# Cogito2012/OpenTAL

Hardware: AMD Instinct MI355X
Metric: clips/sec training step, 256-frame THUMOS14 clips (higher is better)
Workload: dtype bf16

## Files before the change

opental_amd/csrc/conv_gemm.hip:

```cpp
#include "common.h"
#include "conv_index.h"
#include "conv_select.h"
#include <cstdlib>
#include <cstring>
#include <mutex>
#include <type_traits>

#ifndef OTAL_CONV_PART
#define OTAL_CONV_PART 0
#endif

#include "conv1a_tile.h"
namespace otal_conv {
struct ConvArgs;
__attribute__((visibility("hidden"))) int launch_half(int mode, int kernel, int cw, ConvArgs& a, void* ws, size_t ws_bytes, hipStream_t st);
}

namespace {

constexpr int NT = 256;
enum { EPI_RELU = 1, EPI_ACCUM = 2, NO_STORE = 8, NO_BARRIER = 16, EPI_NPAD8 = 32 };

typedef float f32x16 __attribute__((ext_vector_type(16)));

// ... 573 lines not shown
                    pk.y = pack_bf16x2(rb[8 * h + 2], rb[8 * h + 3]);
                    pk.z = pack_bf16x2(rb[8 * h + 4], rb[8 * h + 5]);
                    pk.w = pack_bf16x2(rb[8 * h + 6], rb[8 * h + 7]);
                    *reinterpret_cast<uint4*>(Bs + b_n * KP + b_kq * B_PER + 8 * h) = pk;
                }
            }
        }
    };

    constexpr int WAVES_N = BN / (32 * WN);
    const int wm0 = (wave / WAVES_N) * (32 * WM);
    const int wn0 = (wave % WAVES_N) * (32 * WN);
    f32x16 acc[WM][WN];
#pragma unroll
    for (int i = 0; i < WM; ++i)
#pragma unroll
        for (int j = 0; j < WN; ++j)
#pragma unroll
            for (int r = 0; r < 16; ++r) acc[i][j][r] = 0.f;

    const int nk = (k_end - k_begin + BK - 1) / BK;
    prep(k_begin, nk > 0);
#pragma unroll
    for (int q = 0; q < A_LOADS; ++q) loadA(q, k_begin, nk > 0);
#pragma unroll
    for (int q = 0; q < B_LOADS; ++q) loadB(q, k_begin, nk > 0);
    store_tiles(0);
    __syncthreads();
    constexpr int NCH = PREC ? 2 : 8;
    constexpr int A_PER_CH = (A_LOADS + NCH - 1) / NCH, B_PER_CH = (B_LOADS + NCH - 1) / NCH;
    for (int it = 0; it < nk; ++it) {
        const int buf = it & 1;
        const bool has_next = it + 1 < nk;
        const int kn = k_begin + (it + 1) * BK;
        prep(kn, has_next);
#pragma unroll
        for (int c = 0; c < NCH; ++c) {
#pragma unroll
            for (int q = 0; q < A_PER_CH; ++q)
                if (c * A_PER_CH + q < A_LOADS) loadA(c * A_PER_CH + q, kn, has_next);
#pragma unroll
            for (int q = 0; q < B_PER_CH; ++q)
                if (c * B_PER_CH + q < B_LOADS) loadB(c * B_PER_CH + q, kn, has_next);
            if constexpr (PREC == 0) {
                const float* as = reinterpret_cast<const float*>(smemA[buf]);
                const float* bs = reinterpret_cast<const float*>(smemB[buf]);
                float av[WM], bv[WN];
                const int kr = 2 * c + (lane >> 5);
#pragma unroll
                for (int i = 0; i < WM; ++i) av[i] = as[kr * LDA + wm0 + i * 32 + (lane & 31)];
#pragma unroll
                for (int j = 0; j < WN; ++j) bv[j] = bs[kr * LDB + wn0 + j * 32 + (lane & 31)];
#pragma unroll
                for (int i = 0; i < WM; ++i)
#pragma unroll
                    for (int j = 0; j < WN; ++j)
                        acc[i][j] = __builtin_amdgcn_mfma_f32_32x32x2f32(av[i], bv[j], acc[i][j], 0, 0, 0);
            } else {
                const unsigned short* as = reinterpret_cast<const unsigned short*>(smemA[buf]);
                const unsigned short* bs = reinterpret_cast<const unsigned short*>(smemB[buf]);
                bf16x8 av[WM], bv[WN];
                const int ko = 16 * c + (lane >> 5) * 8;
#pragma unroll
                for (int i = 0; i < WM; ++i)
                    av[i] = *reinterpret_cast<const bf16x8*>(as + (wm0 + i * 32 + (lane & 31)) * KP + ko);
#pragma unroll
                for (int j = 0; j < WN; ++j)
                    bv[j] = *reinterpret_cast<const bf16x8*>(bs + (wn0 + j * 32 + (lane & 31)) * KP + ko);
#pragma unroll
                for (int i = 0; i < WM; ++i)
#pragma unroll
                    for (int j = 0; j < WN; ++j)
                        acc[i][j] = __builtin_amdgcn_mfma_f32_32x32x16_bf16(av[i], bv[j], acc[i][j], 0, 0, 0);
            }
            __builtin_amdgcn_sched_barrier(0);
        }
        if (!(a.flags & NO_STORE)) store_tiles(buf ^ 1);
        if (!(a.flags & NO_BARRIER)) __syncthreads();
    }

    store_acc<MODE, WM, WN, BM>(a, acc, m0, n0, wm0, wn0, lane, split, reinterpret_cast<float*>(smemA[0]));
}

template <int BM, int WM, int WN, int MODE, int CW, bool KWV = false, bool H = false>
__global__ __launch_bounds__(NT, KWV ? 1 : (BM == 96 ? 4 : (BM == 192 ? 3 : 1))) void conv_gemm_bf16c_kernel(const ConvArgs a) {
    static_assert(!KWV || (CW == 1 && MODE == MODE_FWD && !H), "kw-vector mode");
    constexpr int BN = 128, BK = 32, KP = 40;
    constexpr int ESZ = H ? 2 : 4;
    constexpr int PB = CW == 4 ? 36 : (CW == 2 ? 72 : 0);
    constexpr int B_ROWS = CW == 1 ? BN : (CW - 1) * PB + BN / CW;
    constexpr int A_PIECES = (BM * 4 + NT - 1) / NT;
    constexpr int OPER_BYTES = 2 * (BM + B_ROWS) * KP * 2, EPI_BYTES = H ? BM * (BN * 2 + 16) + BM * 8 : 0;
    __shared__ __attribute__((aligned(16))) unsigned char smem_[OPER_BYTES > EPI_BYTES ? OPER_BYTES : EPI_BYTES];
    unsigned short (*const smA)[BM * KP] = reinterpret_cast<unsigned short (*)[BM * KP]>(smem_);
    unsigned short (*const smB)[B_ROWS * KP] = reinterpret_cast<unsigned short (*)[B_ROWS * KP]>(smem_ + 2 * BM * KP * 2);

    const ConvGeom& g = a.g;
    const ConvFastDiv& fd = a.fd;
    const int tid = threadIdx.x;
    const int lane = tid & 63;
    const int wave = __builtin_amdgcn_readfirstlane(tid >> 6);
    const TileId tile = xcd_tile(true);
    const int m0 = tile.y * BM;
    const int n0 = tile.x * BN;
    const int split = tile.z;
    const int k_begin = split * a.k_per_split;
    const int k_end = min(a.Kp, k_begin + a.k_per_split);
    const int nk = (k_end - k_begin) / BK;

    const float* src = MODE == MODE_FWD ? a.x : a.dy;
    const int cs_bytes = (int)((MODE == MODE_FWD ? g.x_cs : g.y_cs) * ESZ);
    const auto rs = __builtin_amdgcn_make_buffer_rsrc(const_cast<float*>(src), 0, (int)a.src_bytes, 0x00020000);
    const auto rw = __builtin_amdgcn_make_buffer_rsrc(const_cast<unsigned short*>(a.wp), 0, (int)a.wp_bytes, 0x00020000);

    const int b_q = CW == 1 ? (tid & 127) : (CW == 4 ? (tid & 31) : lane);
    const int b_kq = __builtin_amdgcn_readfirstlane(tid >> 7);
    unsigned voff0, vmask, keepL_thr = 0u, keepR_thr = 0u;
    {
        const int n = n0 + CW * b_q;
        Anchor an;
        PosDec pd;
        if constexpr (MODE == MODE_FWD) {
            pd = dec_pos_fd(n < a.N ? n : 0, fd.To, fd.Ho, fd.Wo);
            an = anchor_of_output(g, src, pd, n < a.N);
        } else {
            pd = dec_pos_fd(n < a.N ? n : 0, fd.Ti, fd.Hi, fd.Wi);
            an = anchor_of_input(g, src, pd, n < a.N);
        }
        voff0 = (unsigned)((an.base - src) * ESZ);
        vmask = an.mask;
        if constexpr (CW > 1) {
            voff0 += (unsigned)((CW == 4 ? (lane >> 5) * 4 : 0) * cs_bytes);
            keepL_thr = pd.w == 0 ? 0xffffffffu : 0u;
            keepR_thr = pd.w + CW == g.Wi ? 0xffffffffu : 0u;
        }
    }
    unsigned keepw[KWV ? 8 : 1];
    if constexpr (KWV) {
#pragma unroll
        for (int j = 0; j < 8; ++j) keepw[j] = (vmask >> (16 + j)) & 1u ? 0xffffffffu : 0u;
    }
    unsigned voffA[A_PIECES];
#pragma unroll
    for (int j = 0; j < A_PIECES; ++j) {
        const int p = tid + NT * j;
        voffA[j] = (unsigned)(((m0 + (p >> 2)) * a.Kp + (p & 3) * 8) * 2);
    }

    typedef unsigned u32x2 __attribute__((ext_vector_type(2)));
    typedef unsigned u32x4 __attribute__((ext_vector_type(4)));
    u32x4 ra[A_PIECES];
    float rb[H ? 1 : 16];
    unsigned rh[H ? 16 : 1];
    auto tab_off = [](unsigned long long e) { return H ? (unsigned)((int)(unsigned)e >> 1) : (unsigned)e; };
    auto loadA = [&](int k0) {
#pragma unroll
        for (int j = 0; j < A_PIECES; ++j)
            if ((BM * 4) % NT == 0 || tid + NT * j < BM * 4)
                ra[j] = __builtin_amdgcn_raw_buffer_load_b128(rw, voffA[j], k0 * 2, 0);
    };
    constexpr int NE = CW == 1 ? 2 : 1;
    const unsigned long long* ctab64 = reinterpret_cast<const unsigned long long*>(a.ctab) + (CW == 1 ? b_kq * 2 : wave);
    unsigned long long ce[NE], ce_next[NE];
    auto loadT = [&](int k0) {
#pragma unroll
        for (int h = 0; h < NE; ++h) ce_next[h] = ctab64[(k0 >> 3) + h];
    };
    auto loadB = [&](int h) {
        if constexpr (KWV) {
            const unsigned ex = (unsigned)ce[h], ey = (unsigned)(ce[h] >> 32);
            const unsigned sel = (vmask & ey) == ey ? 0xffffffffu : 0u;
            const unsigned vo = ((voff0 + ex) & sel) | (a.src_bytes & ~sel);
            const Words4 v0 = __builtin_bit_cast(Words4, __builtin_amdgcn_raw_buffer_load_b128(rs, vo, 0, 0));
            const Words4 v1 = __builtin_bit_cast(Words4, __builtin_amdgcn_raw_buffer_load_b128(rs, vo + 16u, 0, 0));
            float* r = rb + 8 * h;
            r[0] = __builtin_bit_cast(float, v0.a); r[1] = __builtin_bit_cast(float, v0.b);
            r[2] = __builtin_bit_cast(float, v0.c); r[3] = __builtin_bit_cast(float, v0.d);
            r[4] = __builtin_bit_cast(float, v1.a); r[5] = __builtin_bit_cast(float, v1.b);
            r[6] = __builtin_bit_cast(float, v1.c); r[7] = __builtin_bit_cast(float, v1.d);
        } else if constexpr (CW == 1) {
            const unsigned ex = tab_off(ce[h]), ey = (unsigned)(ce[h] >> 32);
            const unsigned sel = (vmask & ey) == ey ? 0xffffffffu : 0u;
            const unsigned vo = ((voff0 + ex) & sel) | (a.src_bytes & ~sel);
#pragma unroll
            for (int i = 0; i < 8; ++i) {
                if constexpr (H) rh[8 * h + i] = (unsigned)__builtin_amdgcn_raw_buffer_load_b16(rs, vo, i * cs_bytes, 0);
                else rb[8 * h + i] = __builtin_bit_cast(float, __builtin_amdgcn_raw_buffer_load_b32(rs, vo, i * cs_bytes, 0));
            }
        } else if (h == 0) {
            const unsigned ex = tab_off(ce[0]), ey = (unsigned)(ce[0] >> 32);
            const unsigned eth = ey & 0x8000ffffu;
            const unsigned sel = (vmask & eth) == eth ? 0xffffffffu : 0u;
            const unsigned vo = ((voff0 + ex) & sel) | (a.src_bytes & ~sel);
            constexpr int NL = 16 / CW;
#pragma unroll
            for (int i = 0; i < NL; ++i) {
                if constexpr (H && CW == 4) {
                    const Words2 v = __builtin_bit_cast(Words2, __builtin_amdgcn_raw_buffer_load_b64(rs, vo, i * cs_bytes, 0));
                    rh[2 * i] = v.a; rh[2 * i + 1] = v.b;
                } else if constexpr (H) {
                    rh[i] = __builtin_amdgcn_raw_buffer_load_b32(rs, vo, i * cs_bytes, 0);
                } else if constexpr (CW == 4) {
                    const Words4 v = __builtin_bit_cast(Words4, __builtin_amdgcn_raw_buffer_load_b128(rs, vo, i * cs_bytes, 0));
                    rb[4 * i] = __builtin_bit_cast(float, v.a); rb[4 * i + 1] = __builtin_bit_cast(float, v.b);
                    rb[4 * i + 2] = __builtin_bit_cast(float, v.c); rb[4 * i + 3] = __builtin_bit_cast(float, v.d);
                } else {
                    const Words2 v = __builtin_bit_cast(Words2, __builtin_amdgcn_raw_buffer_load_b64(rs, vo, i * cs_bytes, 0));
                    rb[2 * i] = __builtin_bit_cast(float, v.a); rb[2 * i + 1] = __builtin_bit_cast(float, v.b);
                }
            }
        }
    };
    auto fixB = [&]() {
        if constexpr (KWV) {
#pragma unroll
            for (int h = 0; h < 2; ++h) {
                const unsigned ex = (unsigned)ce[h], ey = (unsigned)(ce[h] >> 32);
                const unsigned sel = (vmask & ey) == ey ? 0xffffffffu : 0u;
                const unsigned vo = ((voff0 + ex) & sel) | (a.src_bytes & ~sel);
                float* r = rb + 8 * h;
#pragma unroll
                for (int j = 0; j < 8; ++j) r[j] = __builtin_bit_cast(float, __float_as_uint(r[j]) & keepw[j]);
                const bool neg = vo >= 0xfffffff0u;
                if (__builtin_amdgcn_ballot_w64(neg) != 0ull) {
#pragma unroll
                    for (int j = 1; j < 8; ++j) {
                        const unsigned v = __builtin_amdgcn_raw_buffer_load_b32(rs, neg ? wrap_add(vo, 4u * j) : a.src_bytes, 0, 0);
                        r[j] = neg ? __builtin_bit_cast(float, v & keepw[j]) : r[j];
                    }
                }
            }
        } else if constexpr (CW > 1 && H) {
            const unsigned ex = tab_off(ce[0]), ey = (unsigned)(ce[0] >> 32);
            const unsigned eth = ey & 0x8000ffffu;
            const unsigned dwb = (ey >> 16) & 0xffu;
            const bool below = (dwb & ((1u << g.pw) - 1u)) != 0u, above = (dwb >> (g.pw + 1)) != 0u;
            const unsigned sneg = (MODE == MODE_FWD ? below : above) ? 0xffffffffu : 0u;
            const unsigned spos = (MODE == MODE_FWD ? above : below) ? 0xffffffffu : 0u;
            const unsigned keepL = ~(keepL_thr & sneg) | 0xffff0000u;
            const unsigned keepR = ~(keepR_thr & spos) | 0x0000ffffu;
            const unsigned sel = (vmask & eth) == eth ? 0xffffffffu : 0u;
            const unsigned vo = ((voff0 + ex) & sel) | (a.src_bytes & ~sel);
            constexpr int NL = 16 / CW, WPL = CW / 2;
#pragma unroll
            for (int i = 0; i < NL; ++i) {
                rh[WPL * i] &= keepL;
                rh[WPL * i + WPL - 1] &= keepR;
            }
            const bool neg = vo >= 0xfffffff0u;
            const unsigned gap = a.src_bytes + 2u - 2u * CW - vo;
            bool any = neg;
#pragma unroll
            for (int i = 0; i < NL; ++i) any = any || (vo < a.src_bytes && gap == (unsigned)(i * cs_bytes));
            if (__builtin_amdgcn_ballot_w64(any) != 0ull) {
#pragma unroll
                for (int i = 0; i < NL; ++i) {
                    const bool fix = neg || (vo < a.src_bytes && gap == (unsigned)(i * cs_bytes));
#pragma unroll
                    for (int w = 0; w < WPL; ++w) {
                        const unsigned lo = __builtin_amdgcn_raw_buffer_load_b16(rs, fix ? wrap_add(vo, 4u * w) : a.src_bytes, i * cs_bytes, 0);
                        const unsigned hi = __builtin_amdgcn_raw_buffer_load_b16(rs, fix ? wrap_add(vo, 4u * w + 2u) : a.src_bytes, i * cs_bytes, 0);
                        unsigned v = lo | (hi << 16);
                        if (w == 0) v &= keepL;
                        if (w == WPL - 1) v &= keepR;
                        rh[WPL * i + w] = fix ? v : rh[WPL * i + w];
                    }
                }
            }
        } else if constexpr (CW > 1) {
            const unsigned ex = (unsigned)ce[0], ey = (unsigned)(ce[0] >> 32);
            const unsigned eth = ey & 0x8000ffffu;
            const unsigned dwb = (ey >> 16) & 0xffu;
            const bool below = (dwb & ((1u << g.pw) - 1u)) != 0u, above = (dwb >> (g.pw + 1)) != 0u;
            const unsigned sneg = (MODE == MODE_FWD ? below : above) ? 0xffffffffu : 0u;
            const unsigned spos = (MODE == MODE_FWD ? above : below) ? 0xffffffffu : 0u;
            const unsigned keepL = ~(keepL_thr & sneg), keepR = ~(keepR_thr & spos);
            const unsigned sel = (vmask & eth) == eth ? 0xffffffffu : 0u;
            const unsigned vo = ((voff0 + ex) & sel) | (a.src_bytes & ~sel);
            constexpr int NL = 16 / CW;
#pragma unroll
            for (int i = 0; i < NL; ++i) {
                rb[CW * i] = __builtin_bit_cast(float, __float_as_uint(rb[CW * i]) & keepL);
                rb[CW * i + CW - 1] = __builtin_bit_cast(float, __float_as_uint(rb[CW * i + CW - 1]) & keepR);
            }
            const bool neg = vo >= 0xfffffff0u;
            if (__builtin_amdgcn_ballot_w64(neg) != 0ull) {
#pragma unroll
                for (int i = 0; i < NL; ++i)
#pragma unroll
                    for (int j = 1; j < CW; ++j) {
                        unsigned v = __builtin_amdgcn_raw_buffer_load_b32(rs, neg ? wrap_add(vo, 4u * j) : a.src_bytes, i * cs_bytes, 0);
                        if (j == CW - 1) v &= keepR;
                        rb[CW * i + j] = neg ? __builtin_bit_cast(float, v) : rb[CW * i + j];
                    }
            }
        }
    };
    auto prow = [&](int n) { return CW == 1 ? n : (n % CW) * PB + n / CW; };
    auto store_tiles = [&](int buf) {
        fixB();
        unsigned short* As = smA[buf];
        unsigned short* Bs = smB[buf];
#pragma unroll
        for (int j = 0; j < A_PIECES; ++j) {
            const int p = tid + NT * j;
            if ((BM * 4) % NT == 0 || p < BM * 4) *reinterpret_cast<u32x4*>(As + (p >> 2) * KP + (p & 3) * 8) = ra[j];
        }
        if constexpr (H && CW == 1) {
#pragma unroll
            for (int h = 0; h < 2; ++h) {
                uint4 pk;
                pk.x = pair_lo(rh[8 * h], rh[8 * h + 1]); pk.y = pair_lo(rh[8 * h + 2], rh[8 * h + 3]);
                pk.z = pair_lo(rh[8 * h + 4], rh[8 * h + 5]); pk.w = pair_lo(rh[8 * h + 6], rh[8 * h + 7]);
                *reinterpret_cast<uint4*>(Bs + b_q * KP + b_kq * 16 + 8 * h) = pk;
            }
        } else if constexpr (H && CW == 4) {
#pragma unroll
            for (int j = 0; j < 4; ++j) {
                u32x2 pk;
                pk[0] = (j & 1) ? pair_hi(rh[j >> 1], rh[2 + (j >> 1)]) : pair_lo(rh[j >> 1], rh[2 + (j >> 1)]);
                pk[1] = (j & 1) ? pair_hi(rh[4 + (j >> 1)], rh[6 + (j >> 1)]) : pair_lo(rh[4 + (j >> 1)], rh[6 + (j >> 1)]);
                *reinterpret_cast<u32x2*>(Bs + (j * PB + b_q) * KP + wave * 8 + (lane >> 5) * 4) = pk;
            }
        } else if constexpr (H) {
#pragma unroll
            for (int j = 0; j < 2; ++j) {
                uint4 pk;
                pk.x = j ? pair_hi(rh[0], rh[1]) : pair_lo(rh[0], rh[1]);
                pk.y = j ? pair_hi(rh[2], rh[3]) : pair_lo(rh[2], rh[3]);
                pk.z = j ? pair_hi(rh[4], rh[5]) : pair_lo(rh[4], rh[5]);
                pk.w = j ? pair_hi(rh[6], rh[7]) : pair_lo(rh[6], rh[7]);
                *reinterpret_cast<uint4*>(Bs + (j * PB + b_q) * KP + wave * 8) = pk;
            }
        } else if constexpr (CW == 1) {
#pragma unroll
            for (int h = 0; h < 2; ++h) {
                uint4 pk;
                pk.x = cvt_pk_bf16(rb[8 * h], rb[8 * h + 1]);
                pk.y = cvt_pk_bf16(rb[8 * h + 2], rb[8 * h + 3]);
                pk.z = cvt_pk_bf16(rb[8 * h + 4], rb[8 * h + 5]);
                pk.w = cvt_pk_bf16(rb[8 * h + 6], rb[8 * h + 7]);
                *reinterpret_cast<uint4*>(Bs + b_q * KP + b_kq * 16 + 8 * h) = pk;
            }
        } else if constexpr (CW == 4) {
#pragma unroll
            for (int j = 0; j < 4; ++j) {
                u32x2 pk;
                pk[0] = cvt_pk_bf16(rb[j], rb[4 + j]);
                pk[1] = cvt_pk_bf16(rb[8 + j], rb[12 + j]);
                *reinterpret_cast<u32x2*>(Bs + (j * PB + b_q) * KP + wave * 8 + (lane >> 5) * 4) = pk;
            }
        } else {
#pragma unroll
            for (int j = 0; j < 2; ++j) {
                uint4 pk;
                pk.x = cvt_pk_bf16(rb[j], rb[2 + j]);
                pk.y = cvt_pk_bf16(rb[4 + j], rb[6 + j]);
                pk.z = cvt_pk_bf16(rb[8 + j], rb[10 + j]);
                pk.w = cvt_pk_bf16(rb[12 + j], rb[14 + j]);
                *reinterpret_cast<uint4*>(Bs + (j * PB + b_q) * KP + wave * 8) = pk;
            }
        }
    };

    constexpr int WAVES_N = BN / (32 * WN);
    const int wm0 = (wave / WAVES_N) * (32 * WM);
    const int wn0 = (wave % WAVES_N) * (32 * WN);
    int brow[WN];
#pragma unroll
    for (int j = 0; j < WN; ++j) brow[j] = prow(wn0 + j * 32 + (lane & 31)) * KP + (lane >> 5) * 8;
    f32x16 acc[WM][WN];
#pragma unroll
    for (int i = 0; i < WM; ++i)
#pragma unroll
        for (int j = 0; j < WN; ++j)
#pragma unroll
            for (int r = 0; r < 16; ++r) acc[i][j][r] = 0.f;

    loadT(k_begin);
#pragma unroll
    for (int h = 0; h < NE; ++h) ce[h] = ce_next[h];
    loadT(k_begin + BK);
    if (nk > 0) {
        loadA(k_begin);
        loadB(0);
        loadB(1);
        store_tiles(0);
    }
    __syncthreads();
    for (int it = 0; it < nk; ++it) {
        const int buf = it & 1;
        const int kn = k_begin + (it + 1) * BK;
#pragma unroll
        for (int h = 0; h < NE; ++h) ce[h] = ce_next[h];
        loadT(k_begin + (it + 2) * BK);
        const unsigned short* as = smA[buf];
        const unsigned short* bs = smB[buf];
#pragma unroll
        for (int c = 0; c < 2; ++c) {
            if (c == 0) { loadA(kn); loadB(0); } else loadB(1);
            bf16x8 av[WM], bv[WN];
#pragma unroll
            for (int i = 0; i < WM; ++i)
                av[i] = *reinterpret_cast<const bf16x8*>(as + (wm0 + i * 32 + (lane & 31)) * KP + 16 * c + (lane >> 5) * 8);
#pragma unroll
            for (int j = 0; j < WN; ++j)
                bv[j] = *reinterpret_cast<const bf16x8*>(bs + brow[j] + 16 * c);
#pragma unroll
            for (int i = 0; i < WM; ++i)
#pragma unroll
                for (int j = 0; j < WN; ++j)
                    acc[i][j] = __builtin_amdgcn_mfma_f32_32x32x16_bf16(av[i], bv[j], acc[i][j], 0, 0, 0);
            __builtin_amdgcn_sched_barrier(0);
        }
        store_tiles(buf ^ 1);
        __syncthreads();
    }
    if constexpr (H) {
        if (a.splits == 1) {
            store_acc_h<MODE, WM, WN, BM, BN>(a, acc, m0, n0, wm0, wn0, lane, smem_, NT);
            return;
        }
    }
    store_acc<MODE, WM, WN, BM>(a, acc, m0, n0, wm0, wn0, lane, split, reinterpret_cast<float*>(smA[0]));
}

template <int BM, int WM, int WN, int CW, bool S2 = false, bool H = false>
__global__ __launch_bounds__(NT) void conv_wgrad_bf16v_kernel(const ConvArgs a) {
    static_assert(!S2 || (CW == 8 && !H), "pair mode works on groups of 8 output positions of fp32 tensors");
    constexpr int BN = 128, BK = 32, KP = 40;
    constexpr int ESZ = H ? 2 : 4;
    constexpr int A_PIECES = H ? (BM * 4 + NT - 1) / NT : BM / 32;
    constexpr int NG = S2 ? 1 : 16 / CW;
    __shared__ __attribute__((aligned(16))) unsigned short smA[2][BM * KP];
    __shared__ __attribute__((aligned(16))) unsigned short smB[2][BN * KP];

    const ConvGeom& g = a.g;
    const ConvFastDiv& fd = a.fd;
    const int tid = threadIdx.x;
    const int lane = tid & 63;
    const int wave = __builtin_amdgcn_readfirstlane(tid >> 6);
    const TileId tile = xcd_tile(false);
    const int m0 = tile.y * BM;
    const int n0 = tile.x * BN;
    const int split = tile.z;
    const int k_begin = split * a.k_per_split;
    const int k_end = min(a.K, k_begin + a.k_per_split);
    const int nk = (k_end - k_begin) / BK;

    const auto rx = __builtin_amdgcn_make_buffer_rsrc(const_cast<float*>(a.x), 0, (int)a.src_bytes, 0x00020000);
    const auto rdy = __builtin_amdgcn_make_buffer_rsrc(const_cast<float*>(a.dy), 0, (int)a.dy_bytes, 0x00020000);

    const int b_n = S2 ? 2 * (tid & 63) : (tid & (BN - 1));
    const int b_kq = __builtin_amdgcn_readfirstlane(S2 ? (tid >> 6) : (tid >> 7));
    unsigned coloff, tbits, thrL = 0u, thrR = 0u;
    int dw0 = 0;
    if constexpr (S2) {
        const int n = min(n0 + b_n, a.N - 2);
        const int row = n >> 3;
        const uint32_t q1 = fd_div(fd.kh, (uint32_t)row);
        const int dh = row - (int)(q1 * fd.kh.d);
        const uint32_t ci = fd_div(fd.kt, q1);
        const int dt = (int)(q1 - ci * fd.kt.d);
        dw0 = n & 6;
        coloff = (unsigned)(((int64_t)ci * g.x_cs + ((int64_t)dt * g.Hi + dh) * g.Wi + dw0) * 4);
        tbits = (1u << dt) | (1u << (8 + dh));
    } else {
        const int n = min(n0 + b_n, a.N - 1);
        const TapDec t = dec_tap_fd(fd, (uint32_t)n);
        coloff = (unsigned)(((int64_t)t.c * g.x_cs + ((int64_t)t.dt * g.Hi + t.dh) * g.Wi + t.dw) * ESZ);
        tbits = (1u << t.dt) | (1u << (8 + t.dh));
        thrL = t.dw < g.pw ? 0xffffffffu : 0u;
        thrR = t.dw > g.pw ? 0xffffffffu : 0u;
    }
    unsigned voffA[A_PIECES];
#pragma unroll
    for (int j = 0; j < A_PIECES; ++j) {
        const int p = tid + NT * j;
        if constexpr (H) {
            const int m = min(m0 + (p >> 2), a.M - 1);
            voffA[j] = (unsigned)(((int64_t)m * g.y_cs + (p & 3) * 8) * 2);
        } else {
            const int m = min(m0 + (p >> 3), a.M - 1);
            voffA[j] = (unsigned)(((int64_t)m * g.y_cs + (p & 7) * 4) * 4);
        }
    }

    Words4 ra[A_PIECES];
    float rb[16];
    unsigned rh[8];
    auto tab_off = [](unsigned long long e) { return H ? (unsigned)((int)(unsigned)e >> 1) : (unsigned)e; };
    auto dy_soff = [&](int k0) {
        const int kc = min(k0, a.K - BK);
        const uint32_t b = fd_div(fd.P, (uint32_t)kc);
        return (int)(((int64_t)b * g.y_bs + (kc - (int)(b * fd.P.d))) * ESZ);
    };
    auto loadA = [&](int k0) {
        const int so = dy_soff(k0);
#pragma unroll
// ... 1376 lines not shown
    float* slab = (second ? a.slab2 : a.slab) + (int64_t)split * a.M * a.N;
#pragma unroll
    for (int r = 0; r < 16; ++r) {
        const int co = co0 + mi * 32 + (r & 3) + 8 * (r >> 2) + 4 * (lane >> 5);
        if (co < g.Cout && ci < g.Cin) {
#pragma unroll
            for (int d = 0; d < KT; ++d) slab[(int64_t)co * a.N + ci * KT + d] = acc[d][r];
        }
    }
}

int launch_wgrad1d(ConvArgs& a, void* ws, size_t ws_bytes, hipStream_t st) {
    const int nchunks = wgrad1d_chunks(a.g), units = a.g.B * nchunks;
    const int upw = units >= 8 ? 4 : units >= 4 ? 2 : 1;
    const int splits = (units + upw - 1) / upw;
    const size_t need = ((size_t)splits * a.M * a.N * sizeof(float) + 255) & ~(size_t)255;
    if (!ws || ws_bytes < need * (a.pair ? 2 : 1)) return OTAL_E_UNSUPPORTED;
    a.splits = splits; a.k_per_split = 0; a.slab = reinterpret_cast<float*>(ws);
    if (a.pair) a.slab2 = reinterpret_cast<float*>(reinterpret_cast<char*>(ws) + need);
    const dim3 grid(splits, a.g.Cin / 64, ((a.g.Cout + 63) / 64) * (a.pair ? 2 : 1));
    if (a.g.kt == 1) hipLaunchKernelGGL(conv_wgrad1d_kernel<1>, grid, dim3(256), 0, st, a, nchunks, units, upw);
    else hipLaunchKernelGGL(conv_wgrad1d_kernel<3>, grid, dim3(256), 0, st, a, nchunks, units, upw);
    if (int e = otal_launch_status()) return e;
    if (int e = launch_splitk_reduce<MODE_WGRAD>(a, st)) return e;
    if (a.pair) {
        ConvArgs b = a;
        b.slab = a.slab2; b.out = a.out2;
        return launch_splitk_reduce<MODE_WGRAD>(b, st);
    }
    return 0;
}

static inline int chunk_vector_width(const ConvGeom& g) {
    if (g.st != 1 || g.sh != 1 || g.sw != 1 || g.nlev > 1) return 1;
    if (g.Wo != g.Wi || (g.kw != 1 && g.kw != 3) || g.pw != (g.kw - 1) / 2) return 1;
    if (g.kt == 1 && g.kh == 1 && g.kw == 1 && g.To == g.Ti && g.Ho == g.Hi && conv_out_positions(g) % 4 == 0)
        return 4;
    if (g.Wi % 4 == 0) return 4;
    if (g.Wi % 2 == 0) return 2;
    return 1;
}

template <int MODE>
static void fill_prep_desc(PrepDesc& d, const ConvArgs& a, int2* ctab, unsigned short* wp) {
    const int C = MODE == MODE_FWD ? a.g.Cin : a.g.Cout;
    const bool kwv = MODE == MODE_FWD && (C % 8) != 0;
    const int BMsel = choose_bm(a.M, !kwv);
    d.ctab = ctab; d.wp = reinterpret_cast<unsigned*>(wp); d.wsrc = a.w; d.g = a.g;
    d.M = a.M; d.Mpad = (a.M + BMsel - 1) / BMsel * BMsel; d.C = C; d.kvol = conv_kvol(a.g);
    d.K = a.K; d.Kp = chunk_kp(a.K); d.nchunk = d.Kp / 8 + CHUNK_PAD; d.kwv = kwv ? 1 : 0; d.natural = a.w_natural; d.mode = MODE;
    d.direct = 0;
    d.fh = make_fastdiv((uint32_t)(d.Kp / 2));
    d.fk = make_fastdiv((uint32_t)d.kvol);
}
static inline unsigned prep_blocks(const PrepDesc& d) {
    if (d.direct) {
        const int64_t pairs = (int64_t)d.Mpad * d.C * 27 / 2;
        if (pairs >= (1LL << 31)) return 0;
        const int64_t blocks = (pairs + 256 * PREP_U - 1) / (256 * PREP_U);
        return (unsigned)(blocks < 2048 ? blocks : 2048);
    }
    const int64_t pairs = (int64_t)d.Mpad * (d.Kp / 2);
    if (pairs >= (1LL << 31)) return 0;
    int64_t blocks = (pairs + 256 * PREP_U - 1) / (256 * PREP_U);
    if (d.mode == MODE_DGRAD && d.natural && d.kvol <= PREP_T_KVOL && !d.kwv) blocks = (int64_t)(d.Mpad / 32) * ((d.Kp + 255) / 256);
    if (blocks < (d.nchunk + 255) / 256) blocks = (d.nchunk + 255) / 256;
    return (unsigned)(blocks > 2048 ? 2048 : blocks);
}
static void launch_prep(const PrepDesc& d, hipStream_t st) {
    if (d.direct) {
        if (d.mode == MODE_FWD) hipLaunchKernelGGL((pack_direct_kernel<MODE_FWD>), dim3(prep_blocks(d)), dim3(256), 0, st, d.wp, d.wsrc, d.M, d.Mpad, d.C, d.natural, d.fh);
        else hipLaunchKernelGGL((pack_direct_kernel<MODE_DGRAD>), dim3(prep_blocks(d)), dim3(256), 0, st, d.wp, d.wsrc, d.M, d.Mpad, d.C, d.natural, d.fh);
        return;
    }
    if (d.mode == MODE_FWD) hipLaunchKernelGGL((prep_chunks_kernel<MODE_FWD>), dim3(prep_blocks(d)), dim3(256), 0, st, d);
    else hipLaunchKernelGGL((prep_chunks_kernel<MODE_DGRAD>), dim3(prep_blocks(d)), dim3(256), 0, st, d);
}

#if OTAL_CONV_PART == 1
typedef short v4s16 __attribute__((ext_vector_type(4)));
#include "conv1x1_stream.inc"
#endif

template <int MODE, bool H = false>
int launch_chunked(ConvArgs& a, void* ws, size_t ws_bytes, hipStream_t st) {
    const int C = MODE == MODE_FWD ? a.g.Cin : a.g.Cout;
    const bool kwv = MODE == MODE_FWD && (C % 8) != 0;
    if (H && (kwv || (a.flags & EPI_ACCUM) || conv_in_positions(a.g) != conv_out_positions(a.g))) return OTAL_E_UNSUPPORTED;
    if (kwv) a.K = a.g.Cin * a.g.kt * a.g.kh * 8;
    const int BMpack = choose_bm(a.M, !kwv);
    int BMsel = BMpack;
    if (H && BMsel == 128) BMsel = 96;
    const int tm = (a.M + BMsel - 1) / BMsel, tn = (a.N + 127) / 128;
    a.Kp = chunk_kp(a.K);
    const size_t tb = chunk_tab_bytes(a.K), wb = chunk_wp_bytes(a.M, BMpack, a.K);
    int2* ctab;
    unsigned short* wp;
    if (a.pre) {
        ctab = reinterpret_cast<int2*>(const_cast<void*>(a.pre));
        wp = reinterpret_cast<unsigned short*>(reinterpret_cast<char*>(const_cast<void*>(a.pre)) + tb);
    } else {
        if (!ws || ws_bytes < tb + wb) return OTAL_E_UNSUPPORTED;
        ctab = reinterpret_cast<int2*>(ws);
        wp = reinterpret_cast<unsigned short*>(reinterpret_cast<char*>(ws) + tb);
        PrepDesc d;
        fill_prep_desc<MODE>(d, a, ctab, wp);
        launch_prep(d, st);
        if (int e = otal_launch_status()) return e;
        ws = reinterpret_cast<char*>(ws) + tb + wb;
        ws_bytes -= tb + wb;
    }
    a.ctab = ctab; a.wp = wp;
#if OTAL_CONV_PART == 1
    if constexpr (H) {
        if (conv1x1_stream_eligible(a.g, MODE)) {
            const int e = launch_conv1x1_stream<MODE>(a, wp, wb, (a.M + BMpack - 1) / BMpack * BMpack, st);
            if (e != OTAL_E_UNSUPPORTED) return e;
        }
    }
#endif
    a.src_bytes = (unsigned)gather_extent_bytes(a.g, MODE, H ? 2 : 4);
    a.wp_bytes = (unsigned)wb;
    a.fd = make_conv_fastdiv(a.g);
    int splits = choose_splits(tm * tn, a.Kp);
    if (splits > 1) {
        const size_t need = (size_t)splits * a.M * a.N * sizeof(float);
        if (ws_bytes < need) {
            splits = (int)(ws_bytes / ((size_t)a.M * a.N * sizeof(float)));
            if (splits < 2) splits = 1;
        }
    }
    const int kps = ((a.Kp + splits - 1) / splits + 31) / 32 * 32;
    splits = (a.Kp + kps - 1) / kps;
    a.splits = splits;
    a.k_per_split = kps;
    a.slab = splits > 1 ? (float*)ws : nullptr;
    set_epilogue_extents<MODE>(a);
    const dim3 grid(tn, tm, splits);
    const int cw = chunk_vector_width(a.g);
#define OTAL_LAUNCH_C(BM_, WM_, WN_)                                                                                   \
    do {                                                                                                               \
        if (cw == 4) hipLaunchKernelGGL((conv_gemm_bf16c_kernel<BM_, WM_, WN_, MODE, 4, false, H>), grid, dim3(NT), 0, st, a);   \
        else if (cw == 2) hipLaunchKernelGGL((conv_gemm_bf16c_kernel<BM_, WM_, WN_, MODE, 2, false, H>), grid, dim3(NT), 0, st, a); \
        else hipLaunchKernelGGL((conv_gemm_bf16c_kernel<BM_, WM_, WN_, MODE, 1, false, H>), grid, dim3(NT), 0, st, a);           \
    } while (0)
    if constexpr (MODE == MODE_FWD && !H) {
        if (kwv) {
            if (BMsel == 128) hipLaunchKernelGGL((conv_gemm_bf16c_kernel<128, 2, 2, MODE_FWD, 1, true>), grid, dim3(NT), 0, st, a);
            else if (BMsel == 96) hipLaunchKernelGGL((conv_gemm_bf16c_kernel<96, 3, 1, MODE_FWD, 1, true>), grid, dim3(NT), 0, st, a);
            else if (BMsel == 64) hipLaunchKernelGGL((conv_gemm_bf16c_kernel<64, 2, 1, MODE_FWD, 1, true>), grid, dim3(NT), 0, st, a);
            else hipLaunchKernelGGL((conv_gemm_bf16c_kernel<32, 1, 1, MODE_FWD, 1, true>), grid, dim3(NT), 0, st, a);
        }
    }
    if (kwv) {
    } else if (BMsel == 192) OTAL_LAUNCH_C(192, 6, 1);
    else if (BMsel == 128) { if constexpr (!H) OTAL_LAUNCH_C(128, 2, 2); }
    else if (BMsel == 96) OTAL_LAUNCH_C(96, 3, 1);
    else if (BMsel == 64) OTAL_LAUNCH_C(64, 2, 1);
    else OTAL_LAUNCH_C(32, 1, 1);
#undef OTAL_LAUNCH_C
    if (int e = otal_launch_status()) return e;
    if (splits > 1) {
        return launch_splitk_reduce<MODE, H>(a, st);
    }
    return 0;
}

template <bool H = false>
int launch_wgrad_vector(ConvArgs& a, int cw, void* ws, size_t ws_bytes, hipStream_t st) {
    const bool pair = a.g.sw == 2;
    if (H && pair) return OTAL_E_UNSUPPORTED;
    if (pair) {
        a.N = a.g.Cin * a.g.kt * a.g.kh * 8;
        a.flags |= EPI_NPAD8;
    }
    const int BMsel = choose_bm(a.M);
    const int tm = (a.M + BMsel - 1) / BMsel, tn = (a.N + 127) / 128;
    const size_t tb = ptab_bytes(a.g, cw);
    a.fd = make_conv_fastdiv(a.g);
    a.P = conv_out_positions(a.g);
    a.src_bytes = (unsigned)gather_extent_bytes(a.g, MODE_FWD, H ? 2 : 4);
    a.dy_bytes = (unsigned)gather_extent_bytes(a.g, MODE_DGRAD, H ? 2 : 4);
    int2* ptab;
    if (a.pre) {
        ptab = reinterpret_cast<int2*>(const_cast<void*>(a.pre));
    } else {
        if (!ws || ws_bytes < tb) return OTAL_E_UNSUPPORTED;
        ptab = reinterpret_cast<int2*>(ws);
        const int ngroups = a.K / cw, npad = ngroups + PTAB_PAD;
        hipLaunchKernelGGL(build_pos_table_kernel, dim3((npad + 255) / 256), dim3(256), 0, st, ptab, a.g, a.fd, cw, ngroups, npad);
        if (int e = otal_launch_status()) return e;
        ws = reinterpret_cast<char*>(ws) + tb;
        ws_bytes -= tb;
    }
    a.ptab = ptab;
    int splits = choose_splits(tm * tn, a.K, 1, true);
    if (splits > 1) {
        const size_t need = (size_t)splits * a.M * a.N * sizeof(float);
        if (ws_bytes < need) {
            splits = (int)(ws_bytes / ((size_t)a.M * a.N * sizeof(float)));
            if (splits < 2) splits = 1;
        }
    }
    const int kps = ((a.K + splits - 1) / splits + 31) / 32 * 32;
    splits = (a.K + kps - 1) / kps;
    a.splits = splits;
    a.k_per_split = kps;
    a.slab = splits > 1 ? (float*)ws : nullptr;
    set_epilogue_extents<MODE_WGRAD>(a);
    const dim3 grid(tn, tm, splits);
#define OTAL_LAUNCH_W(BM_, WM_, WN_)                                                                                   \
    do {                                                                                                               \
        if (cw == 8) hipLaunchKernelGGL((conv_wgrad_bf16v_kernel<BM_, WM_, WN_, 8, false, H>), grid, dim3(NT), 0, st, a);        \
        else if (cw == 4) hipLaunchKernelGGL((conv_wgrad_bf16v_kernel<BM_, WM_, WN_, 4, false, H>), grid, dim3(NT), 0, st, a);   \
        else hipLaunchKernelGGL((conv_wgrad_bf16v_kernel<BM_, WM_, WN_, 2, false, H>), grid, dim3(NT), 0, st, a);                \
    } while (0)
    if constexpr (!H) {
        if (pair) {
            if (BMsel == 128) hipLaunchKernelGGL((conv_wgrad_bf16v_kernel<128, 2, 2, 8, true>), grid, dim3(NT), 0, st, a);
            else if (BMsel == 96) hipLaunchKernelGGL((conv_wgrad_bf16v_kernel<96, 3, 1, 8, true>), grid, dim3(NT), 0, st, a);
            else if (BMsel == 64) hipLaunchKernelGGL((conv_wgrad_bf16v_kernel<64, 2, 1, 8, true>), grid, dim3(NT), 0, st, a);
            else hipLaunchKernelGGL((conv_wgrad_bf16v_kernel<32, 1, 1, 8, true>), grid, dim3(NT), 0, st, a);
        }
    }
    if (pair) {
    } else if (BMsel == 192) OTAL_LAUNCH_W(192, 6, 1);
    else if (BMsel == 128) OTAL_LAUNCH_W(128, 2, 2);
// ... 490 lines not shown
```

opental_amd/csrc/options.h:

```cpp
#pragma once

struct OtalOption { const char* name; int dflt; };
constexpr OtalOption OTAL_OPTIONS[] = {
    {"OTAL_CONV_1A_NOTILE", 0},           {"OTAL_CONV_1A_WGS", 0},
    {"OTAL_CONV_DIRECT_MINTILES", 140},   {"OTAL_CONV_DIRECT_MINTILES512", 512},
    {"OTAL_CONV_DIRECT_XPF2", 3},         {"OTAL_CONV_NO1A", 0},
    {"OTAL_CONV_NO1AW", 0},               {"OTAL_CONV_NO1DTILE", 0},
    {"OTAL_CONV_NO1X1STREAM", 0},         {"OTAL_CONV_NODIRECT", 0},
    {"OTAL_CONV_NOPROJ", 0},              {"OTAL_CONV_NOPROJW", 0},
    {"OTAL_CONV_NOW1D", 0},               {"OTAL_CONV_NOW1X1", 0},
    {"OTAL_CONV_NOWDIRECT", 0},           {"OTAL_LOSS_NOSTAGE", 0},
    {"OTAL_POOL_NO133", 0},               {"OTAL_POOL_NOROWS", 0},
    {"OTAL_W1A_SPLITS", 0},               {"OTAL_WDIRECT_BLOCKS", 0},
};
constexpr int OTAL_NUM_OPTIONS = sizeof(OTAL_OPTIONS) / sizeof(OTAL_OPTIONS[0]);
constexpr bool otal_streq(const char* a, const char* b) { return *a == *b && (*a == 0 || otal_streq(a + 1, b + 1)); }
constexpr int otal_option_index(const char* name, int i = 0) {
    return i == OTAL_NUM_OPTIONS ? -1 : otal_streq(OTAL_OPTIONS[i].name, name) ? i : otal_option_index(name, i + 1);
}
int* otal_option_slot(int index);
#define OTAL_OPT(name) ([]() -> int {                                                                              \
    constexpr int index_ = otal_option_index(name);                                                              \
    static_assert(index_ >= 0, "unknown option " name " (options.h: OTAL_OPTIONS)");                               \
    static int* const slot_ = otal_option_slot(index_);                                                          \
    return *slot_;                                                                                               \
}())
```

Before: 1001.

## Add deeper register prefetch pipeline to chunked conv GEMM for small grids

```diff
diff --git a/opental_amd/csrc/conv_gemm.hip b/opental_amd/csrc/conv_gemm.hip
--- a/opental_amd/csrc/conv_gemm.hip
+++ b/opental_amd/csrc/conv_gemm.hip
@@ -679,9 +679,10 @@
     store_acc<MODE, WM, WN, BM>(a, acc, m0, n0, wm0, wn0, lane, split, reinterpret_cast<float*>(smemA[0]));
 }
 
-template <int BM, int WM, int WN, int MODE, int CW, bool KWV = false, bool H = false>
-__global__ __launch_bounds__(NT, KWV ? 1 : (BM == 96 ? 4 : (BM == 192 ? 3 : 1))) void conv_gemm_bf16c_kernel(const ConvArgs a) {
+template <int BM, int WM, int WN, int MODE, int CW, bool KWV = false, bool H = false, int PF = 1>
+__global__ __launch_bounds__(NT, KWV ? 1 : (PF > 1 ? (BM == 128 ? 1 : 2) : (BM == 96 ? 4 : (BM == 192 ? 3 : 1)))) void conv_gemm_bf16c_kernel(const ConvArgs a) {
     static_assert(!KWV || (CW == 1 && MODE == MODE_FWD && !H), "kw-vector mode");
+    static_assert(PF >= 1 && PF <= 3 && (PF == 1 || !KWV), "prefetch depth");
     constexpr int BN = 128, BK = 32, KP = 40;
     constexpr int ESZ = H ? 2 : 4;
     constexpr int PB = CW == 4 ? 36 : (CW == 2 ? 72 : 0);
@@ -746,11 +747,15 @@
 
     typedef unsigned u32x2 __attribute__((ext_vector_type(2)));
     typedef unsigned u32x4 __attribute__((ext_vector_type(4)));
-    u32x4 ra[A_PIECES];
-    float rb[H ? 1 : 16];
-    unsigned rh[H ? 16 : 1];
+    u32x4 ra_[PF][A_PIECES];
+    float rb_[PF][H ? 1 : 16];
+    unsigned rh_[PF][H ? 16 : 1];
+    using Set0 = std::integral_constant<int, 0>;
+    using Set1 = std::integral_constant<int, (PF > 1 ? 1 : 0)>;
+    using Set2 = std::integral_constant<int, (PF > 2 ? 2 : 0)>;
     auto tab_off = [](unsigned long long e) { return H ? (unsigned)((int)(unsigned)e >> 1) : (unsigned)e; };
-    auto loadA = [&](int k0) {
+    auto loadA = [&](int k0, auto set) {
+        u32x4* const ra = ra_[decltype(set)::value];
 #pragma unroll
         for (int j = 0; j < A_PIECES; ++j)
             if ((BM * 4) % NT == 0 || tid + NT * j < BM * 4)
@@ -758,12 +763,17 @@
     };
     constexpr int NE = CW == 1 ? 2 : 1;
     const unsigned long long* ctab64 = reinterpret_cast<const unsigned long long*>(a.ctab) + (CW == 1 ? b_kq * 2 : wave);
-    unsigned long long ce[NE], ce_next[NE];
+    unsigned long long ce_[PF][NE], ce_next[NE];
+    unsigned long long (&ce)[NE] = ce_[0];
     auto loadT = [&](int k0) {
 #pragma unroll
         for (int h = 0; h < NE; ++h) ce_next[h] = ctab64[(k0 >> 3) + h];
     };
-    auto loadB = [&](int h) {
+    auto loadB = [&](int h, auto set) {
+        constexpr int S = decltype(set)::value;
+        float* const rb = rb_[S];
+        unsigned* const rh = rh_[S];
+        const unsigned long long* const ce = ce_[S];
         if constexpr (KWV) {
             const unsigned ex = (unsigned)ce[h], ey = (unsigned)(ce[h] >> 32);
             const unsigned sel = (vmask & ey) == ey ? 0xffffffffu : 0u;
@@ -808,7 +818,12 @@
             }
         }
     };
-    auto fixB = [&]() {
+    auto settle = [](auto& v) { if constexpr (PF > 1) asm volatile("" : "+v"(v)); };
+    auto fixB = [&](auto set) {
+        constexpr int S = decltype(set)::value;
+        float* const rb = rb_[S];
+        unsigned* const rh = rh_[S];
+        const unsigned long long* const ce = ce_[S];
         if constexpr (KWV) {
 #pragma unroll
             for (int h = 0; h < 2; ++h) {
@@ -861,6 +876,7 @@
                         if (w == 0) v &= keepL;
                         if (w == WPL - 1) v &= keepR;
                         rh[WPL * i + w] = fix ? v : rh[WPL * i + w];
+                        settle(rh[WPL * i + w]);
                     }
                 }
             }
@@ -889,13 +905,18 @@
                         unsigned v = __builtin_amdgcn_raw_buffer_load_b32(rs, neg ? wrap_add(vo, 4u * j) : a.src_bytes, i * cs_bytes, 0);
                         if (j == CW - 1) v &= keepR;
                         rb[CW * i + j] = neg ? __builtin_bit_cast(float, v) : rb[CW * i + j];
+                        settle(rb[CW * i + j]);
                     }
             }
         }
     };
     auto prow = [&](int n) { return CW == 1 ? n : (n % CW) * PB + n / CW; };
-    auto store_tiles = [&](int buf) {
-        fixB();
+    auto store_tiles = [&](int buf, auto set) {
+        constexpr int S = decltype(set)::value;
+        fixB(set);
+        const u32x4* const ra = ra_[S];
+        const float* const rb = rb_[S];
+        const unsigned* const rh = rh_[S];
         unsigned short* As = smA[buf];
         unsigned short* Bs = smB[buf];
 #pragma unroll
@@ -974,44 +995,117 @@
 #pragma unroll
             for (int r = 0; r < 16; ++r) acc[i][j][r] = 0.f;
 
-    loadT(k_begin);
-#pragma unroll
-    for (int h = 0; h < NE; ++h) ce[h] = ce_next[h];
-    loadT(k_begin + BK);
-    if (nk > 0) {
-        loadA(k_begin);
-        loadB(0);
-        loadB(1);
-        store_tiles(0);
-    }
-    __syncthreads();
-    for (int it = 0; it < nk; ++it) {
-        const int buf = it & 1;
-        const int kn = k_begin + (it + 1) * BK;
+    if constexpr (PF == 1) {
+        loadT(k_begin);
 #pragma unroll
         for (int h = 0; h < NE; ++h) ce[h] = ce_next[h];
-        loadT(k_begin + (it + 2) * BK);
-        const unsigned short* as = smA[buf];
-        const unsigned short* bs = smB[buf];
-#pragma unroll
-        for (int c = 0; c < 2; ++c) {
-            if (c == 0) { loadA(kn); loadB(0); } else loadB(1);
-            bf16x8 av[WM], bv[WN];
-#pragma unroll
-            for (int i = 0; i < WM; ++i)
-                av[i] = *reinterpret_cast<const bf16x8*>(as + (wm0 + i * 32 + (lane & 31)) * KP + 16 * c + (lane >> 5) * 8);
-#pragma unroll
-            for (int j = 0; j < WN; ++j)
-                bv[j] = *reinterpret_cast<const bf16x8*>(bs + brow[j] + 16 * c);
-#pragma unroll
-            for (int i = 0; i < WM; ++i)
+        loadT(k_begin + BK);
+        if (nk > 0) {
+            loadA(k_begin, Set0{});
+            loadB(0, Set0{});
+            loadB(1, Set0{});
+            store_tiles(0, Set0{});
+        }
+        __syncthreads();
+        for (int it = 0; it < nk; ++it) {
+            const int buf = it & 1;
+            const int kn = k_begin + (it + 1) * BK;
+#pragma unroll
+            for (int h = 0; h < NE; ++h) ce[h] = ce_next[h];
+            loadT(k_begin + (it + 2) * BK);
+            const unsigned short* as = smA[buf];
+            const unsigned short* bs = smB[buf];
+#pragma unroll
+            for (int c = 0; c < 2; ++c) {
+                if (c == 0) { loadA(kn, Set0{}); loadB(0, Set0{}); } else loadB(1, Set0{});
+                bf16x8 av[WM], bv[WN];
+#pragma unroll
+                for (int i = 0; i < WM; ++i)
+                    av[i] = *reinterpret_cast<const bf16x8*>(as + (wm0 + i * 32 + (lane & 31)) * KP + 16 * c + (lane >> 5) * 8);
 #pragma unroll
                 for (int j = 0; j < WN; ++j)
-                    acc[i][j] = __builtin_amdgcn_mfma_f32_32x32x16_bf16(av[i], bv[j], acc[i][j], 0, 0, 0);
-            __builtin_amdgcn_sched_barrier(0);
-        }
-        store_tiles(buf ^ 1);
+                    bv[j] = *reinterpret_cast<const bf16x8*>(bs + brow[j] + 16 * c);
+#pragma unroll
+                for (int i = 0; i < WM; ++i)
+#pragma unroll
+                    for (int j = 0; j < WN; ++j)
+                        acc[i][j] = __builtin_amdgcn_mfma_f32_32x32x16_bf16(av[i], bv[j], acc[i][j], 0, 0, 0);
+                __builtin_amdgcn_sched_barrier(0);
+            }
+            store_tiles(buf ^ 1, Set0{});
+            __syncthreads();
+        }
+    } else {
+        auto kof = [&](int s) { return k_begin + max(min(s, nk - 1), 0) * BK; };
+        (void)ce; (void)ce_next; (void)loadT;
+        unsigned long long tv[NE];
+        int tv0 = 0;
+        auto loadTV = [&](int s0) {
+            tv0 = s0;
+#pragma unroll
+            for (int h = 0; h < NE; ++h) {
+                tv[h] = ctab64[(kof(s0 + lane) >> 3) + h];
+                asm volatile("" : "+v"(tv[h]));
+            }
+        };
+        auto entries = [&](int s, auto set) {
+            const int sc = max(min(s, nk - 1), 0);
+            if ((sc >> 6) != (tv0 >> 6)) loadTV(sc & ~63);
+#pragma unroll
+            for (int h = 0; h < NE; ++h) {
+                const unsigned lo = (unsigned)__builtin_amdgcn_readlane((int)(unsigned)tv[h], sc - tv0);
+                const unsigned hi = (unsigned)__builtin_amdgcn_readlane((int)(unsigned)(tv[h] >> 32), sc - tv0);
+                ce_[decltype(set)::value][h] = ((unsigned long long)hi << 32) | lo;
+            }
+        };
+        auto issue = [&](int k0, auto set) { loadA(k0, set); loadB(0, set); loadB(1, set); };
+        loadTV(0);
+        entries(0, Set0{});
+        entries(1, Set1{});
+        if constexpr (PF > 2) entries(2, Set2{});
+        if (nk > 0) {
+            issue(kof(0), Set0{});
+            issue(kof(1), Set1{});
+            if constexpr (PF > 2) issue(kof(2), Set2{});
+            store_tiles(0, Set0{});
+        }
         __syncthreads();
+        auto kstep = [&](int it, auto cur, auto nxt) {
+            const int buf = it & 1;
+            const int kn = kof(it + PF);
+            entries(it + PF, cur);
+            const unsigned short* as = smA[buf];
+            const unsigned short* bs = smB[buf];
+#pragma unroll
+            for (int c = 0; c < 2; ++c) {
+                if (c == 0) { loadA(kn, cur); loadB(0, cur); } else loadB(1, cur);
+                bf16x8 av[WM], bv[WN];
+#pragma unroll
+                for (int i = 0; i < WM; ++i)
+                    av[i] = *reinterpret_cast<const bf16x8*>(as + (wm0 + i * 32 + (lane & 31)) * KP + 16 * c + (lane >> 5) * 8);
+#pragma unroll
+                for (int j = 0; j < WN; ++j)
+                    bv[j] = *reinterpret_cast<const bf16x8*>(bs + brow[j] + 16 * c);
+#pragma unroll
+                for (int i = 0; i < WM; ++i)
+#pragma unroll
+                    for (int j = 0; j < WN; ++j)
+                        acc[i][j] = __builtin_amdgcn_mfma_f32_32x32x16_bf16(av[i], bv[j], acc[i][j], 0, 0, 0);
+                __builtin_amdgcn_sched_barrier(0);
+            }
+            store_tiles(buf ^ 1, nxt);
+            __syncthreads();
+        };
+        int it = 0;
+        for (; it + PF <= nk; it += PF) {
+            kstep(it, Set0{}, Set1{});
+            if constexpr (PF == 2) kstep(it + 1, Set1{}, Set0{});
+            else { kstep(it + 1, Set1{}, Set2{}); kstep(it + 2, Set2{}, Set0{}); }
+        }
+        if (it < nk) {
+            kstep(it, Set0{}, Set1{});
+            if constexpr (PF == 3) { if (it + 1 < nk) kstep(it + 1, Set1{}, Set2{}); }
+        }
     }
     if constexpr (H) {
         if (a.splits == 1) {
@@ -2554,6 +2648,24 @@
 #include "conv1x1_stream.inc"
 #endif
 
+constexpr int CHUNK_PF_MAX_WGS = 256;
+constexpr bool chunk_has_deep(int BM, int CW, int MODE, bool H) {
+    if (BM == 32) return true;
+    if (H || BM == 192) return false;
+    if (CW == 1) return true;
+    if (CW == 4) return BM == 128 || (BM == 96 ? MODE == MODE_DGRAD : MODE == MODE_FWD);
+    return false;
+}
+static inline int chunk_pf_depth(int BM, bool H) { return H || BM == 192 ? 1 : 2; }
+template <int BM, int WM, int WN, int MODE, int CW, bool H>
+static void launch_chunked_pf(int pf, dim3 grid, hipStream_t st, const ConvArgs& a) {
+    if constexpr (chunk_has_deep(BM, CW, MODE, H)) {
+        if (pf >= 3) { hipLaunchKernelGGL((conv_gemm_bf16c_kernel<BM, WM, WN, MODE, CW, false, H, 3>), grid, dim3(NT), 0, st, a); return; }
+        if (pf == 2) { hipLaunchKernelGGL((conv_gemm_bf16c_kernel<BM, WM, WN, MODE, CW, false, H, 2>), grid, dim3(NT), 0, st, a); return; }
+    }
+    hipLaunchKernelGGL((conv_gemm_bf16c_kernel<BM, WM, WN, MODE, CW, false, H>), grid, dim3(NT), 0, st, a);
+}
+
 template <int MODE, bool H = false>
 int launch_chunked(ConvArgs& a, void* ws, size_t ws_bytes, hipStream_t st) {
     const int C = MODE == MODE_FWD ? a.g.Cin : a.g.Cout;
@@ -2610,11 +2722,13 @@
     set_epilogue_extents<MODE>(a);
     const dim3 grid(tn, tm, splits);
     const int cw = chunk_vector_width(a.g);
+    int pf = OTAL_OPT("OTAL_CONV_CHUNK_PF");
+    if (pf == 0) pf = (int64_t)tm * tn * splits <= CHUNK_PF_MAX_WGS ? chunk_pf_depth(BMsel, H) : 1;
 #define OTAL_LAUNCH_C(BM_, WM_, WN_)                                                                                   \
     do {                                                                                                               \
-        if (cw == 4) hipLaunchKernelGGL((conv_gemm_bf16c_kernel<BM_, WM_, WN_, MODE, 4, false, H>), grid, dim3(NT), 0, st, a);   \
-        else if (cw == 2) hipLaunchKernelGGL((conv_gemm_bf16c_kernel<BM_, WM_, WN_, MODE, 2, false, H>), grid, dim3(NT), 0, st, a); \
-        else hipLaunchKernelGGL((conv_gemm_bf16c_kernel<BM_, WM_, WN_, MODE, 1, false, H>), grid, dim3(NT), 0, st, a);           \
+        if (cw == 4) launch_chunked_pf<BM_, WM_, WN_, MODE, 4, H>(pf, grid, st, a);                                    \
+        else if (cw == 2) launch_chunked_pf<BM_, WM_, WN_, MODE, 2, H>(pf, grid, st, a);                               \
+        else launch_chunked_pf<BM_, WM_, WN_, MODE, 1, H>(pf, grid, st, a);                                            \
     } while (0)
     if constexpr (MODE == MODE_FWD && !H) {
         if (kwv) {
diff --git a/opental_amd/csrc/options.h b/opental_amd/csrc/options.h
--- a/opental_amd/csrc/options.h
+++ b/opental_amd/csrc/options.h
@@ -3,6 +3,7 @@
 struct OtalOption { const char* name; int dflt; };
 constexpr OtalOption OTAL_OPTIONS[] = {
     {"OTAL_CONV_1A_NOTILE", 0},           {"OTAL_CONV_1A_WGS", 0},
+    {"OTAL_CONV_CHUNK_PF", 0},
     {"OTAL_CONV_DIRECT_MINTILES", 140},   {"OTAL_CONV_DIRECT_MINTILES512", 512},
     {"OTAL_CONV_DIRECT_XPF2", 3},         {"OTAL_CONV_NO1A", 0},
     {"OTAL_CONV_NO1AW", 0},               {"OTAL_CONV_NO1DTILE", 0},
```

After: 1001. Within noise of the previous version (-0.0%).
